# microsoft/NOTSOFAR1-Challenge

Measured on AMD Instinct MI355X. Metric: CSS real-time-factor (sep. audio sec/wall sec) on 7-ch 16 kHz, higher is better.
Workload: dtype f32 (float32 operands on v_mfma_f32_32x32x2_f32 in every Linear layer, attention product and transform: the reference's own operand precision; MVDR covariance / solve f64)

## Files before the change

include/css_mi355.h:

```cpp
#ifndef CSS_MI355_H
#define CSS_MI355_H

#include <stddef.h>
#include <stdint.h>

#ifdef __cplusplus
extern "C" {
#endif
#if defined(__GNUC__) || defined(__clang__)
#pragma GCC visibility push(default)
#endif

typedef struct css_ctx* css_handle_t;

typedef enum css_status {
    CSS_OK = 0,
    CSS_ERR_INVALID_ARG = -1,
    CSS_ERR_HIP = -2,
    CSS_ERR_ZERO_WEIGHT = -3,
    CSS_ERR_MASK_FLOOR = -4,
    CSS_ERR_SHAPE = -5,
    CSS_ERR_STATE = -6,
    CSS_ERR_NO_DEVICE = -7,
    CSS_ERR_WEIGHT_WINDOW = -8,
// ... 79 lines not shown
    CSS_BUF_ACT_FINAL = 11,
    CSS_BUF_Y = 12,
    CSS_BUF_WAV = 13,
    CSS_BUF_HIDDEN = 14,
    CSS_BUF_WTA_OVERRIDE = 15,
    CSS_BUF_LEVEL = 16
} css_buffer;

const char* css_version(void);
const char* css_last_error(css_handle_t h);
int css_device_count(void);

int64_t css_blob_num_floats(const CssModelDesc* desc);

int css_create(const CssModelDesc* desc, const float* blob_host, int64_t blob_floats, int device,
               void* stream, int32_t max_batch_segments, css_handle_t* out);
int css_destroy(css_handle_t h);
int css_get_stream(css_handle_t h, void** stream_out);
int css_set_lanes(css_handle_t h, int lanes);
int css_get_lanes(css_handle_t h);
enum css_tuning {
    CSS_TUNE_TAIL_PIECES = 0,
    CSS_TUNE_OUT_MAPPED = 1,
    CSS_TUNE_TAIL_PER_UNIT = 2,
    CSS_TUNE_MVDR_ON_LANES = 3,
    CSS_TUNE_PIPELINE_DEVICE = 4,
    CSS_TUNE_GROUP_LANES = 5,
    CSS_TUNE_GROUP_TRANSFORM_ON_MAIN = 6,
    CSS_TUNE_GROUP_MVDR_ON_LANES = 7,
    CSS_TUNE_GROUP_OUT_DMA = 8,
    CSS_TUNE_F32_GEMM = 9,
    CSS_TUNE_SPLIT_BATCH_ROWS = 10,
    CSS_TUNE_F32_LANE_ROWS = 11,
    CSS_TUNE_COUNT = 12
};
int css_set_tuning(css_handle_t h, int which, int value);
int css_host_alloc(size_t bytes, void** out);
int css_host_free(void* p);

int css_plan(const CssModelDesc* desc, const CssRunCfg* cfg, int64_t n_samples, CssPlan* out);
int css_pit_scan(const double* costs, int64_t n_boundaries, int32_t num_spks, int32_t* perms);

typedef struct CssCfgSeconds {
    double segment_size_sec;
    double hop_size_sec;
    double seg_weight_m0_sec;
    double seg_weight_m1_sec;
    double activity_dilation_sec;
    double activity_erosion_sec;
    double activity_th;
    double mask_floor_db;
    int32_t mc_mvdr, stitching_loss , stitching_input , normalize_segment_power;
} CssCfgSeconds;
int css_make_run_cfg(const CssModelDesc* desc, const CssCfgSeconds* cfg, int32_t fs, CssRunCfg* out, float* windows, int64_t cap);

int css_run(css_handle_t h, const float* pcm_host, int64_t n_samples, int32_t n_ch, const CssRunCfg* cfg,
            float* wav_host, int64_t wav_capacity_per_stream);
int css_run_enqueue(css_handle_t h, const float* pcm_host, int64_t n_samples, int32_t n_ch, const CssRunCfg* cfg,
                    float* wav_host, int64_t cap);
int css_set_queue_group(css_handle_t h, int max_sessions);
int css_wait(css_handle_t h);
int css_wait_sessions(css_handle_t h, int64_t n);
int css_run_device(css_handle_t h, const float* pcm_dev, int64_t n_samples, int32_t n_ch, const CssRunCfg* cfg,
                   float* wav_dev, int64_t wav_capacity_per_stream);
int css_run_pcm16(css_handle_t h, const int16_t* const* planes_host, int64_t n_samples, int32_t n_ch, const CssRunCfg* cfg,
                  int16_t* wav_pcm16_host, int64_t wav_capacity_per_stream, float* peaks_host);
int css_run_enqueue_pcm16(css_handle_t h, const int16_t* const* planes_host, int64_t n_samples, int32_t n_ch, const CssRunCfg* cfg,
// ... 129 lines not shown
```

notsofar1-challenge_amd/_lib.py:

```python
from __future__ import annotations

import ctypes as C
import os
from typing import Optional

import numpy as np

_HERE = os.path.dirname(os.path.abspath(__file__))
LIB_PATH = os.environ.get("CSS_MI355_LIBRARY") or os.path.join(_HERE, "libcss_mi355.so")


class CssLibraryError(RuntimeError):
    pass


class CssError(RuntimeError):
    def __init__(self, code: int, text: str):
        super().__init__(f"css_mi355 error {code}: {text}")
        self.code = code
        self.text = text


CSS_OK, CSS_ERR_INVALID_ARG, CSS_ERR_HIP, CSS_ERR_ZERO_WEIGHT, CSS_ERR_MASK_FLOOR = 0, -1, -2, -3, -4
CSS_ERR_SHAPE, CSS_ERR_STATE, CSS_ERR_NO_DEVICE, CSS_ERR_WEIGHT_WINDOW, CSS_ERR_RANGE = -5, -6, -7, -8, -9
# ... 359 lines not shown
        blob = np.ascontiguousarray(blob, dtype=np.float32)
        need = lib.css_blob_num_floats(C.byref(self._cdesc))
        if need != blob.size:
            raise CssError(CSS_ERR_INVALID_ARG, f"weight blob has {blob.size} floats, library expects {need}")
        h = C.c_void_p()
        rc = lib.css_create(C.byref(self._cdesc), _np_ptr(blob), blob.size, int(device),
                            C.c_void_p(stream) if stream else None, int(max_batch_segments), C.byref(h))
        if rc != CSS_OK:
            raise CssError(rc, lib.css_last_error(None).decode("utf-8", "replace"))
        self.h = h
        self.device = device

    def close(self):
        if getattr(self, "h", None):
            self.lib.css_destroy(self.h)
            self.h = None

    def __del__(self):
        try:
            self.close()
        except Exception:
            pass

    def stream_ptr(self) -> int:
        p = C.c_void_p()
        check(self.h, self.lib.css_get_stream(self.h, C.byref(p)))
        return int(p.value or 0)

    def set_lanes(self, lanes: int):
        check(self.h, self.lib.css_set_lanes(self.h, int(lanes)))

    def set_tuning(self, which, value: int):
        idx = {"tail_pieces": 0, "out_mapped": 1, "tail_per_unit": 2, "mvdr_on_lanes": 3, "pipeline_device": 4,
               "group_lanes": 5, "group_transform_on_main": 6, "group_mvdr_on_lanes": 7, "group_out_dma": 8, "f32_gemm": 9, "split_batch_rows": 10, "f32_lane_rows": 11}[which] if isinstance(which, str) else int(which)
        check(self.h, self.lib.css_set_tuning(self.h, idx, int(value)))

    def set_queue_group(self, max_sessions: int):
        check(self.h, self.lib.css_set_queue_group(self.h, int(max_sessions)))

    def lanes(self) -> int:
        return int(self.lib.css_get_lanes(self.h))

    def run(self, pcm: np.ndarray, cfg: RunCfg, out: Optional[np.ndarray] = None) -> np.ndarray:
        pcm = np.ascontiguousarray(pcm, dtype=np.float32)
        n, c = pcm.shape
        p = plan(self.desc, cfg, n)
        if out is None:
            out = np.empty((self.desc.num_spks, p.n_out), dtype=np.float32)
        assert out.dtype == np.float32 and out.ndim == 2 and out.shape[0] == self.desc.num_spks and out.shape[1] >= p.n_out \
            and out.strides[1] == 4
        check(self.h, self.lib.css_run(self.h, _np_ptr(pcm), n, c, C.byref(cfg.c), _np_ptr(out), out.strides[0] // 4))
        return out[:, :p.n_out]

    def run_enqueue(self, pcm: np.ndarray, cfg: RunCfg, out: np.ndarray) -> np.ndarray:
        assert pcm.dtype == np.float32 and pcm.flags.c_contiguous and pcm.ndim == 2
        n, c = pcm.shape
        p = plan(self.desc, cfg, n)
        assert out.dtype == np.float32 and out.ndim == 2 and out.shape[0] == self.desc.num_spks and out.shape[1] >= p.n_out \
            and out.strides[1] == 4
        self._queued_keep = getattr(self, "_queued_keep", []) + [(pcm, out, cfg)]
        check(self.h, self.lib.css_run_enqueue(self.h, _np_ptr(pcm), n, c, C.byref(cfg.c), _np_ptr(out), out.strides[0] // 4))
        return out[:, :p.n_out]

    def wait(self):
        try:
            check(self.h, self.lib.css_wait(self.h))
        finally:
# ... 293 lines not shown
```

notsofar1-challenge_amd/csrc/api_ctx.hpp:

```cpp
#pragma once
#include "../../include/css_mi355.h"

#include <algorithm>
#include <cmath>
#include <cstdlib>
#include <cstdio>
#include <cstring>
#include <chrono>
#include <functional>
#include <string>
#include <vector>

#include <dlfcn.h>
#include <mutex>

#include "kernels.hpp"
#include "lsap.hpp"

using namespace css;

enum ProfCat : int {
    CSS_PROF_DEINTERLEAVE = 0, CSS_PROF_STFT, CSS_PROF_FEATURES, CSS_PROF_LINEAR, CSS_PROF_LAYERNORM, CSS_PROF_ATTENTION,
    CSS_PROF_CONV, CSS_PROF_SCM, CSS_PROF_MVDR_SOLVE, CSS_PROF_BEAMFORM, CSS_PROF_PIT, CSS_PROF_OLA_MASKS, CSS_PROF_GATE,
    CSS_PROF_OLA_STFT, CSS_PROF_ISTFT_GEMM, CSS_PROF_WAVE_OLA, CSS_PROF_ENCODE, CSS_PROF_COUNT
// ... 85 lines not shown
    bool split_ok = true;
    float* wsplit = nullptr;
    float* dft_split = nullptr;
    float* wfrag = nullptr;
    float* dft_tiled = nullptr;
    float* head_tiled = nullptr;
    DevBuf pe_frag[2];
    int pe_frag_T[2] = {0, 0};
    float* stft_tab = nullptr;
    bool fft512 = true;
    float* dft_fwd = nullptr;
    int Lp = 0, ovl = 2;
    float* dft_inv_t = nullptr;

    std::vector<float> w_on_device;
    DevBuf pcm_in, feat, hx, hu, ht, qkv, qkf, ctxb, masks, segw, stage, in16, pcm_f, enc, level, mel_tab, mel_work;
    static constexpr int MAX_GROUP = 8;
    std::vector<SessState> slots;
    int group_limit = MAX_GROUP;
    static constexpr int MAX_LANES = 4;
    int lanes = 3;
    hipStream_t lane_stream[MAX_LANES] = {};
    hipEvent_t ev_fork = nullptr, ev_join[MAX_LANES] = {};
    DevBuf lfeat[MAX_LANES], lhx[MAX_LANES], lhu[MAX_LANES], lht[MAX_LANES], lqkv[MAX_LANES], lqkf[MAX_LANES], lctx[MAX_LANES];
    int64_t last_batch_tokens = 0;
    int mel_bands = 0;
    unsigned int* range_flag_dev = nullptr;
    unsigned int* range_flag_host = nullptr;
    bool range_fallback = true;
    int64_t range_fallbacks = 0;
    int range_last = 0;
    hipStream_t copy_stream = nullptr;
    hipStream_t tail_stream = nullptr;
    int tune[CSS_TUNE_COUNT] = {1, 0, 0, 1, 0, 2, 1, 0, 1, 0, 24576, 14000};
    const void* mapped_key = nullptr;
    void* mapped_val = nullptr;
    int queued = 0;
    int64_t pass_no = 0;
    hipEvent_t pcm_free[2] = {nullptr, nullptr};
    hipEvent_t pass_end[4] = {nullptr, nullptr, nullptr, nullptr};
    hipEvent_t level_free[2] = {nullptr, nullptr};
    hipEvent_t tail_end = nullptr;
    bool tail_pending = false;
    bool piped_now = false;
    int last_piped = -1;
    struct QueuedSession {
        const float* pcm; int64_t n; int32_t n_ch; CssRunCfg cfg; float* wav; int64_t cap;
        std::vector<const int16_t*> planes; int16_t* wav16; float* peaks;
        float* wav_mapped;
        std::vector<float> w;
        QueuedSession(const float* pcm_, const int16_t* const* planes_, int64_t n_, int32_t n_ch_, const CssRunCfg& c, float* wav_,
                      int16_t* wav16_, float* peaks_, int64_t cap_, float* mapped_)
            : pcm(pcm_), n(n_), n_ch(n_ch_), cfg(c), wav(wav_), cap(cap_), wav16(wav16_), peaks(peaks_), wav_mapped(mapped_) {
            if (planes_) planes.assign(planes_, planes_ + n_ch_);
            const size_t T = (size_t)std::max(c.segment_frames, 0);
            w.resize(3 * T);
            if (T && c.w_first && c.w_mid && c.w_last) {
                std::memcpy(w.data(), c.w_first, T * sizeof(float));
                std::memcpy(w.data() + T, c.w_mid, T * sizeof(float));
                std::memcpy(w.data() + 2 * T, c.w_last, T * sizeof(float));
            }
        }
        bool pcm16() const { return !planes.empty(); }
        CssRunCfg own_cfg() const {
            CssRunCfg c = cfg;
            const size_t T = w.size() / 3;
            c.w_first = w.data(); c.w_mid = w.data() + T; c.w_last = w.data() + 2 * T;
// ... 153 lines not shown
```

notsofar1-challenge_amd/csrc/api_stages.hip:

```cpp
#include "api_ctx.hpp"

int check_run_args(css_handle_t h, int64_t n_samples, int32_t n_ch, const CssRunCfg* cfg, CssPlan* plan_out) {
    if (!h || !cfg) return fail(h, CSS_ERR_INVALID_ARG, "null argument");
    if (n_ch != h->d.num_mics)
        return fail(h, CSS_ERR_SHAPE, "input has " + std::to_string(n_ch) + " channels, the model expects " + std::to_string(h->d.num_mics));
    if (!cfg->w_first || !cfg->w_mid || !cfg->w_last) return fail(h, CSS_ERR_INVALID_ARG, "segment weights missing");
    if (cfg->mask_floor > 1.0f || cfg->mask_floor < 0.f) return fail(h, CSS_ERR_MASK_FLOOR, "mask_floor_db must be <= 0");
    const int T = cfg->segment_frames, hop = cfg->hop_frames;
    if (T < 2 || T > CSS_MAX_SEGMENT_FRAMES)
        return fail(h, CSS_ERR_INVALID_ARG, "segment_frames must be in [2, " + std::to_string(CSS_MAX_SEGMENT_FRAMES) + "]");
    if (cfg->stitching_loss < 0 || cfg->stitching_loss > 1 || cfg->stitching_input < 0 || cfg->stitching_input > 1)
        return fail(h, CSS_ERR_INVALID_ARG, "unexpected stitching_loss / stitching_input");
    if (hop <= 0 || hop >= T) return fail(h, CSS_ERR_INVALID_ARG, "hop_frames must satisfy 1 <= hop < T (at least one frame of overlap for the stitching cost, css.py:276)");
    CssPlan p{};
    if (plan_impl(h->d, *cfg, n_samples, &p) != CSS_OK) return fail(h, CSS_ERR_INVALID_ARG, "bad segment configuration");
    if (p.zero_weight) return fail(h, CSS_ERR_ZERO_WEIGHT, "zero weights found. check hop_size, segment_size or m0, m1");
    *plan_out = p;
    return CSS_OK;
}

int begin_impl(css_handle_t h, int64_t n_samples, int32_t n_ch, const CssRunCfg* cfg) {
    CssPlan p{};
    int rc0 = check_run_args(h, n_samples, n_ch, cfg, &p);
    if (rc0 != CSS_OK) return rc0;
// ... 229 lines not shown
                       const float* w2, const float* b2) {
            if (with_ln) { CSS_PROF(CSS_PROF_LAYERNORM, st); launch_layernorm(xin, sp ? nullptr : u, sp ? u : nullptr, lnw, lnb, M, D, 0, st); }
            gemm(h, lin(u, D, w1, b1, t1, FF, FF, D, ACT_RELU, FF), st);
            GemmArgs g = lin(t1, FF, w2, b2, x, D, D, FF, ACT_NONE, 0);
            g.residual = xin; g.ldr = D; g.alpha = 0.5f;
            gemm(h, g, st);
        };
        ffn(l == 0, x, b.ffi_ln_w, b.ffi_ln_b, b.ffi_w1, b.ffi_b1, b.ffi_w2, b.ffi_b2);
        { CSS_PROF(CSS_PROF_LAYERNORM, st); launch_layernorm(x, sp ? nullptr : u, sp ? u : nullptr, b.att_ln_w, b.att_ln_b, M, D, 0, st); }
        const bool long_seg = T > 512 || css_force_long_path();
        {
            GemmArgs g = lin(u, D, b.wqkv, b.bqkv, qkv, 3 * D, 3 * D, D, ACT_NONE, long_seg ? 0 : 3 * D);
            if (sp && !long_seg) { g.frag_out = qkf; g.frag_D = D; g.frag_T = T; g.frag_heads = d.attention_heads; g.frag_invT = 1.0f / T; }
            gemm(h, g, st);
        }
        {
            CSS_PROF(CSS_PROF_ATTENTION, st);
            if (long_seg) {
                if (!launch_relpos_attention_long(qkv, W.pe_k, cb, nb, T, D, d.attention_heads, d.maxlen, sp, st)) return CSS_ERR_INVALID_ARG;
            } else {
                launch_relpos_attention(qkv, sp ? qkf : nullptr, (const float*)h->pe_frag[sp].p, cb, nb, T, D, d.attention_heads, d.maxlen, sp, sp, st);
            }
        }
        {
            GemmArgs g = lin(cb, D, b.wo, b.bo, x, D, D, D, ACT_NONE, 0);
            g.residual = x; g.ldr = D; g.alpha = 1.f;
            gemm(h, g, st);
        }
        const float* xc = cb;
        bool ffo_ln = false;
        {
        CSS_PROF(CSS_PROF_CONV, st);
        if (!launch_conv_module(x, cb, b.conv_ln_w, b.conv_ln_b, b.pw, b.dw_wt, b.dw_b, b.bn_alpha, b.bn_beta, b.ffo_ln_w,
                                b.ffo_ln_b, sp ? nullptr : u, sp ? u : nullptr, nb, T, D, d.kernel_size, st)) {
            launch_ln_glu(x, u, b.conv_ln_w, b.conv_ln_b, b.pw, M, D, st);
            launch_dwconv(u, x, b.dw_wt, b.dw_b, b.bn_alpha, b.bn_beta, b.pw, nb, T, D, d.kernel_size, st);
            xc = x;
            ffo_ln = true;
        }
        }
        ffn(ffo_ln, xc, b.ffo_ln_w, b.ffo_ln_b, b.ffo_w1, b.ffo_b1, b.ffo_w2, b.ffo_b2);
        if (!last) {
            const BlockWeights& nb_ = W.blocks[l + 1];
            { CSS_PROF(CSS_PROF_LAYERNORM, st); launch_layernorm2(x, x, b.fin_ln_w, b.fin_ln_b, sp ? nullptr : u, sp ? u : nullptr, nb_.ffi_ln_w, nb_.ffi_ln_b, M, D, st); }
        } else {
            { CSS_PROF(CSS_PROF_LAYERNORM, st); launch_layernorm(x, x, sp ? u : nullptr, b.fin_ln_w, b.fin_ln_b, M, D, 0, st); }
        }
    }
    if (ph_hi <= d.num_blocks) return CSS_OK;
    GemmArgs g{};
    const int nout = F * (d.num_spks + d.num_nois);
    if (sp) {
        g.A = u; g.lda = D; g.strideA = 0;
        g.B = h->head_tiled; g.ldb = D; g.strideB = 0; g.b_tiled = 1;
        g.C = io.masks + s0 * T; g.ldc = io.mask_ld; g.strideC = 0; g.c_transposed = 1;
        g.M = M; g.N = nout; g.K = D; g.batch = 1;
        g.bias = W.head_b; g.bias_along_m = 0; g.act = ACT_SIGMOID; g.residual = nullptr; g.alpha = 1.f;
        g.split_in = 1; g.concurrent = concurrent ? 1 : 0;
        g.range_flag = h->range_flag_dev;
    } else {
        g.A = WS(W.head_w); g.lda = D; g.strideA = 0;
        g.B = sp ? u : x; g.ldb = D; g.strideB = 0;
        g.C = io.masks + s0 * T; g.ldc = io.mask_ld; g.strideC = 0;
        g.M = nout; g.N = M; g.K = D; g.batch = 1;
        g.bias = W.head_b; g.bias_along_m = 1; g.act = ACT_SIGMOID; g.residual = nullptr; g.alpha = 1.f;
        g.split_in = sp;
        g.range_flag = sp ? h->range_flag_dev : nullptr;
// ... 573 lines not shown
```

notsofar1-challenge_amd/csrc/encoder.hip:

```cpp
#include "kernels.hpp"
#include "split_f16.hpp"

namespace css {

typedef float f32x16 __attribute__((ext_vector_type(16)));
typedef _Float16 f16x8 __attribute__((ext_vector_type(8)));

template <int CTRL>
__device__ __forceinline__ float dpp_addf(float v) {
    return v + __int_as_float(__builtin_amdgcn_update_dpp(0, __float_as_int(v), CTRL, 0xf, 0xf, false));
}
__device__ __forceinline__ float wave_sum(float v) {
    v = dpp_addf<0xB1>(v);
    v = dpp_addf<0x4E>(v);
    v = dpp_addf<0x141>(v);
    v = dpp_addf<0x140>(v);
    const float r0 = __int_as_float(__builtin_amdgcn_readlane(__float_as_int(v), 0));
    const float r1 = __int_as_float(__builtin_amdgcn_readlane(__float_as_int(v), 16));
    const float r2 = __int_as_float(__builtin_amdgcn_readlane(__float_as_int(v), 32));
    const float r3 = __int_as_float(__builtin_amdgcn_readlane(__float_as_int(v), 48));
    return (r0 + r1) + (r2 + r3);
}

#ifndef CSS_LN_ROWS
// ... 144 lines not shown
#pragma clang loop unroll(full)
    for (int p = 0; p < RUN + TAPS - 1; ++p) {
        const int t = t0 + p - PAD;
        const float v = (t >= 0 && t < T) ? zs[(int64_t)t * D] : 0.f;
#pragma clang loop unroll(full)
        for (int j = (p - (TAPS - 1) > 0 ? p - (TAPS - 1) : 0); j <= (p < RUN - 1 ? p : RUN - 1); ++j)
            acc[j] = fmaf(wk[p - j], v, acc[j]);
    }
    const float bb = dwb[ch], al = alpha[ch], be = beta[ch], w2 = pw[4], c2 = pw[5];
    float* hs = h + (int64_t)seg * T * D + ch;
#pragma unroll
    for (int j = 0; j < RUN; ++j) {
        const int t = t0 + j;
        if (t < T) {
            const float y = fmaxf((acc[j] + bb) * al + be, 0.f);
            hs[(int64_t)t * D] += w2 * y + c2;
        }
    }
}

void launch_dwconv(const float* z, float* h, const float* dw_wt, const float* dw_b, const float* bn_alpha,
                   const float* bn_beta, const float* pw, int nseg, int T, int D, int taps, hipStream_t s) {
    constexpr int RUN = 31;
    const int runs = (T + RUN - 1) / RUN;
    const dim3 grid((D + 255) / 256, nseg * runs), block(256);
    if (taps == 33)
        hipLaunchKernelGGL((dwconv_kernel<33, RUN>), grid, block, 0, s, z, h, dw_wt, dw_b, bn_alpha, bn_beta, pw, T, D, runs);
    else if (taps == 31)
        hipLaunchKernelGGL((dwconv_kernel<31, RUN>), grid, block, 0, s, z, h, dw_wt, dw_b, bn_alpha, bn_beta, pw, T, D, runs);
    else if (taps == 17)
        hipLaunchKernelGGL((dwconv_kernel<17, RUN>), grid, block, 0, s, z, h, dw_wt, dw_b, bn_alpha, bn_beta, pw, T, D, runs);
}

template <int NV, int TAPS, int RUN, int HV>
__global__ __launch_bounds__(256 * NV * HV) void conv_module_kernel(const float* __restrict__ x_in, float* __restrict__ x_out,
                                                              const float* __restrict__ lnw, const float* __restrict__ lnb,
                                                              const float* __restrict__ pw, const float* __restrict__ wt,
                                                              const float* __restrict__ dwb, const float* __restrict__ alpha,
                                                              const float* __restrict__ beta,
                                                              const float* __restrict__ ln2w, const float* __restrict__ ln2b,
                                                              float* __restrict__ z, float* __restrict__ zs, int T, int runs_per_seg) {
    constexpr int D = 256 * NV, PAD = (TAPS - 1) / 2, ROWS = RUN + TAPS - 1, NW = 4 * NV * HV, JH = (RUN + HV - 1) / HV;
    extern __shared__ __attribute__((aligned(16))) float tile[];
    const int item = css_xcd_item((int)blockIdx.x, (int)gridDim.x);
    const int seg = item / runs_per_seg, run = item % runs_per_seg;
    const int t0 = run * RUN;
    const int wave = threadIdx.x >> 6, lane = threadIdx.x & 63;
    const float p0 = pw[0], p1 = pw[1], p2 = pw[2], p3 = pw[3];
    const int ch = threadIdx.x % D, j0 = (threadIdx.x / D) * JH;
    float wk[TAPS];
#pragma clang loop unroll(full)
    for (int k = 0; k < TAPS; ++k) wk[k] = wt[k * D + ch];
    const float bb = dwb[ch], al = alpha[ch], be_ = beta[ch], w2 = pw[4], c2 = pw[5];
    const float* xs = x_in + (int64_t)seg * T * D + ch;
    float xres[JH];
#pragma clang loop unroll(full)
    for (int j = 0; j < JH; ++j) xres[j] = xs[(int64_t)min(t0 + j0 + j, T - 1) * D];
    constexpr int RPW = (ROWS + NW - 1) / NW;
    float4 v[RPW][NV];
#pragma unroll
    for (int i = 0; i < RPW; ++i) {
        const int p = wave + i * NW, t = t0 + p - PAD;
        const bool ok = p < ROWS && t >= 0 && t < T;
        const float4* xr = reinterpret_cast<const float4*>(x_in + ((int64_t)seg * T + (ok ? t : 0)) * D);
#pragma unroll
        for (int j = 0; j < NV; ++j) v[i][j] = ok ? xr[lane + 64 * j] : make_float4(0.f, 0.f, 0.f, 0.f);
    }
#pragma unroll
    for (int i = 0; i < RPW; ++i) {
        const int p = wave + i * NW, t = t0 + p - PAD;
        if (p >= ROWS) break;
        float4* dst = reinterpret_cast<float4*>(tile + p * D);
        if (t < 0 || t >= T) {
#pragma unroll
            for (int j = 0; j < NV; ++j) dst[lane + 64 * j] = make_float4(0.f, 0.f, 0.f, 0.f);
            continue;
        }
        float s = 0.f;
#pragma unroll
        for (int j = 0; j < NV; ++j) s += (v[i][j].x + v[i][j].y) + (v[i][j].z + v[i][j].w);
        const float mean = wave_sum(s) * (1.0f / D);
        float q = 0.f;
#pragma unroll
        for (int j = 0; j < NV; ++j) {
            v[i][j].x -= mean; v[i][j].y -= mean; v[i][j].z -= mean; v[i][j].w -= mean;
            q += (v[i][j].x * v[i][j].x + v[i][j].y * v[i][j].y) + (v[i][j].z * v[i][j].z + v[i][j].w * v[i][j].w);
        }
        const float rstd = 1.0f / sqrtf(wave_sum(q) * (1.0f / D) + 1e-5f);
#pragma unroll
        for (int j = 0; j < NV; ++j) {
            const float4 g = reinterpret_cast<const float4*>(lnw)[lane + 64 * j];
            const float4 be = reinterpret_cast<const float4*>(lnb)[lane + 64 * j];
            float o[4] = {v[i][j].x * rstd * g.x + be.x, v[i][j].y * rstd * g.y + be.y, v[i][j].z * rstd * g.z + be.z,
                          v[i][j].w * rstd * g.w + be.w};
#pragma unroll
            for (int e = 0; e < 4; ++e) {
                const float z = p2 * o[e] + p3;
                o[e] = (p0 * o[e] + p1) * __builtin_amdgcn_rcpf(1.0f + __builtin_amdgcn_exp2f(z * -1.44269504088896341f));
            }
            dst[lane + 64 * j] = make_float4(o[0], o[1], o[2], o[3]);
        }
    }
    __syncthreads();
    float acc[JH];
#pragma clang loop unroll(full)
    for (int j = 0; j < JH; ++j) acc[j] = 0.f;
#pragma clang loop unroll(full)
    for (int pp = 0; pp < JH + TAPS - 1; ++pp) {
        const float zv = tile[min(j0 + pp, ROWS - 1) * D + ch];
#pragma clang loop unroll(full)
        for (int j = (pp - (TAPS - 1) > 0 ? pp - (TAPS - 1) : 0); j <= (pp < JH - 1 ? pp : JH - 1); ++j)
            acc[j] = fmaf(wk[pp - j], zv, acc[j]);
    }
    __syncthreads();
#pragma unroll
    for (int j = 0; j < JH; ++j) {
        const float y = fmaxf((acc[j] + bb) * al + be_, 0.f);
        if (j0 + j < RUN) tile[(j0 + j) * D + ch] = xres[j] + (w2 * y + c2);
    }
    __syncthreads();
    for (int j = wave; j < RUN && t0 + j < T; j += NW) {
        const int64_t row = (int64_t)seg * T + t0 + j;
        float4 r[NV];
        float s = 0.f;
#pragma unroll
        for (int i = 0; i < NV; ++i) {
            r[i] = reinterpret_cast<const float4*>(tile + j * D)[lane + 64 * i];
            reinterpret_cast<float4*>(x_out + row * D)[lane + 64 * i] = r[i];
            s += (r[i].x + r[i].y) + (r[i].z + r[i].w);
        }
        if (!z && !zs) continue;
        const float mean = wave_sum(s) * (1.0f / D);
        float q = 0.f;
#pragma unroll
        for (int i = 0; i < NV; ++i) {
            r[i].x -= mean; r[i].y -= mean; r[i].z -= mean; r[i].w -= mean;
            q += (r[i].x * r[i].x + r[i].y * r[i].y) + (r[i].z * r[i].z + r[i].w * r[i].w);
        }
        const float rstd = 1.0f / sqrtf(wave_sum(q) * (1.0f / D) + 1e-5f);
#pragma unroll
        for (int i = 0; i < NV; ++i) {
            const float4 g = reinterpret_cast<const float4*>(ln2w)[lane + 64 * i];
            const float4 be = reinterpret_cast<const float4*>(ln2b)[lane + 64 * i];
            const float4 o = make_float4(r[i].x * rstd * g.x + be.x, r[i].y * rstd * g.y + be.y, r[i].z * rstd * g.z + be.z,
                                         r[i].w * rstd * g.w + be.w);
            if (z) reinterpret_cast<float4*>(z + row * D)[lane + 64 * i] = o;
            if (zs) split_store4(reinterpret_cast<_Float16*>(zs + row * D), 4 * (lane + 64 * i), o.x, o.y, o.z, o.w);
        }
    }
}

bool launch_conv_module(const float* x_in, float* x_out, const float* ln_w, const float* ln_b, const float* pw,
                        const float* dw_wt, const float* dw_b, const float* bn_alpha, const float* bn_beta,
                        const float* ln2_w, const float* ln2_b, float* z, float* z_split, int nseg, int T,
                        int D, int taps, hipStream_t s) {
#ifndef CSS_CONV_RUN
#define CSS_CONV_RUN 31
#endif
    constexpr int RUN = CSS_CONV_RUN;
    if (taps != 33 || (D != 256 && D != 512)) return false;
    const int runs = (T + RUN - 1) / RUN;
    const size_t lds = (size_t)(RUN + 32) * D * sizeof(float);
    const void* fn = D == 512 ? reinterpret_cast<const void*>(&conv_module_kernel<2, 33, RUN, 2>)
                              : reinterpret_cast<const void*>(&conv_module_kernel<1, 33, RUN, 2>);
    if (hipFuncSetAttribute(fn, hipFuncAttributeMaxDynamicSharedMemorySize, 160 * 1024) != hipSuccess) {
        (void)hipGetLastError();
        return false;
    }
    if (D == 512)
        hipLaunchKernelGGL((conv_module_kernel<2, 33, RUN, 2>), dim3(nseg * runs), dim3(1024), lds, s, x_in, x_out, ln_w, ln_b, pw, dw_wt,
                           dw_b, bn_alpha, bn_beta, ln2_w, ln2_b, z, z_split, T, runs);
    else
        hipLaunchKernelGGL((conv_module_kernel<1, 33, RUN, 2>), dim3(nseg * runs), dim3(512), lds, s, x_in, x_out, ln_w, ln_b, pw, dw_wt,
                           dw_b, bn_alpha, bn_beta, ln2_w, ln2_b, z, z_split, T, runs);
    return true;
}

template <int NJT, bool QKS, bool FRAG, int W>
__global__ __launch_bounds__(64 * W, (NJT <= 7 ? 2 : 1)) void relpos_attn_kernel(const float* __restrict__ qkv, const float* __restrict__ qkf,
                                                         const float* __restrict__ pe,
                                                         float* __restrict__ ctx, int T, int D, int maxlen,
                                                         int split_out, int heads, int n_items) {
    constexpr int DK = 64;
    constexpr int LDR = 98;
    const int wv = W > 1 ? __builtin_amdgcn_readfirstlane((int)(threadIdx.x >> 6)) : 0;
    __shared__ __attribute__((aligned(16))) float lds_all[W][32 * LDR];
    float (&lds)[32 * LDR] = lds_all[wv];
    const int item = css_xcd_item((int)blockIdx.x, (int)gridDim.x) * W + wv;
    if (item >= n_items) return;
    const int qt = item % NJT, head = (item / NJT) % heads, seg = item / (NJT * heads);
    const int lane = threadIdx.x & 63, c = lane & 31, h = lane >> 5;
    const int ld = 3 * D;
    const float* qb = qkv + (int64_t)seg * T * ld + head * DK;
    const float* kb = qb + D;
    const float* vb = qb + 2 * D;
    const int i0 = qt * 32;
    const int iq = min(i0 + c, T - 1);

    float4 q[8];
#define CSS_ATT_LOAD8(dst, rowptr)                                                                      \
    _Pragma("unroll") for (int ch = 0; ch < 8; ++ch)                                                    \
        dst[ch] = *reinterpret_cast<const float4*>((rowptr) + (QKS ? ((ch >> 2) * 32 + ((ch >> 1) & 1) * 8 + (ch & 1) * 16) : 8 * ch) + 4 * h);
    const float4* qkt = reinterpret_cast<const float4*>(qkf) +
                        ((int64_t)(seg * heads + head) * NJT) * (2 * 8 * 64) + lane;
    if constexpr (FRAG) {
#pragma unroll
        for (int ch = 0; ch < 8; ++ch) q[ch] = qkt[(qt * 2 + 0) * 512 + ch * 64];
// ... 430 lines not shown
```

notsofar1-challenge_amd/csrc/kernels.hpp:

```cpp
#pragma once
#include <hip/hip_runtime.h>
#include <stdint.h>

namespace css {

enum GemmAct : int { ACT_NONE = 0, ACT_RELU = 1, ACT_SIGMOID = 2 };

struct GemmArgs {
    const float* A; int64_t lda; int64_t strideA;
    const float* B; int64_t ldb; int64_t strideB;
    float* C; int64_t ldc; int64_t strideC;
    int M, N, K, batch;
    const float* bias;
    int bias_along_m;
    int act;
    const float* residual;
    int64_t ldr;
    float alpha;
    int split_in;
    int split_out;
    int b_tiled;
    int b_frag32;
    const float* B_rows;
    int concurrent;
    int nt_store;
    float* frag_out;
    int frag_D, frag_T, frag_heads;
    float frag_invT;
    int tile_rows;
    int narrow_epilogue;
    unsigned int* range_flag;
    int layout;
    int m_fastest;
    int c_transposed;
};
void launch_gemm(const GemmArgs& g, hipStream_t s);
bool launch_gemm_f32(const GemmArgs& g, hipStream_t s, int forced_tm);
void launch_f32_fragments(const float* src, int64_t ld_src, float* dst, int N, int K, hipStream_t s);
void launch_gemm_split(const GemmArgs& g, hipStream_t s);
void launch_gemm_split_wd(const GemmArgs& g, hipStream_t s);
void launch_split_convert_tiled(const float* src, int64_t ld_src, float* dst, int N, int K, hipStream_t s);
void launch_split_convert(const float* src, int64_t ld_src, float* dst, int64_t rows, int K, int Kp, hipStream_t s);

void launch_layernorm(const float* x, float* y, float* y_split, const float* w, const float* b, int rows, int D,
                      int relu, hipStream_t s);
void launch_layernorm2(const float* x, float* y, const float* w1, const float* b1, float* z, float* z_split,
                       const float* w2, const float* b2, int rows, int D, hipStream_t s);
void launch_ln_glu(const float* x, float* z, const float* w, const float* b, const float* pw, int rows, int D,
                   hipStream_t s);
void launch_dwconv(const float* z, float* h, const float* dw_wt, const float* dw_b, const float* bn_alpha,
                   const float* bn_beta, const float* pw, int nseg, int T, int D, int taps, hipStream_t s);
bool launch_conv_module(const float* x_in, float* x_out, const float* ln_w, const float* ln_b, const float* pw,
                        const float* dw_wt, const float* dw_b, const float* bn_alpha, const float* bn_beta,
                        const float* ln2_w, const float* ln2_b, float* z, float* z_split, int nseg, int T,
                        int D, int taps, hipStream_t s);
inline int pe_fragment_tiles(int T) { return 2 * ((T + 31) / 32); }
void launch_pe_fragments(const float* pe, float* frag, int T, int maxlen, int split, hipStream_t s);
inline int64_t qk_fragment_floats(int64_t nseg, int T, int H) { return nseg * H * ((T + 31) / 32) * 2 * 8 * 64 * 4; }
void launch_relpos_attention(const float* qkv, const float* qk_frag, const float* pe_frag, float* ctx, int nseg, int T, int D,
                             int H, int maxlen, int qk_split, int split_out, hipStream_t s);
bool launch_relpos_attention_long(const float* qkv, const float* pe, float* ctx, int nseg, int T, int D, int H, int maxlen,
                                  int split_out, hipStream_t s);

size_t stft_table_floats();
void stft_build_tables(float* host, int window = 0);
bool launch_stft_fft(const float* x, int64_t x_stride, int C, int64_t t_lo, int64_t t_hi, const float* tables, float* out,
                     int64_t row_ld, hipStream_t s, float* phase = nullptr);

__device__ __forceinline__ int css_xcd_item(int L, int n) {
    const int q = n >> 3, rem = n & 7, xcd = L & 7;
    return xcd * q + (xcd < rem ? xcd : rem) + (L >> 3);
}

#define CSS_PHASE_NEG_REAL (-3.14159250259399414f)
__device__ __forceinline__ float css_phase_of(float re, float im) {
    return (im == 0.f && re < 0.f) ? CSS_PHASE_NEG_REAL : atan2f(im, re);
}

void launch_deinterleave(const float* pcm, float* pcm_cm, int64_t n, int C, int64_t n_pad, int64_t i_lo, int64_t i_hi,
                         int split_out, hipStream_t s);
void launch_pcm_peak_f32(const float* x, int64_t count, unsigned int* peak, hipStream_t s);
void launch_pcm_peak_i16(const int16_t* x, int64_t count, unsigned int* peak, hipStream_t s);
void launch_pcm16_to_float(const int16_t* planes, float* pcm, int64_t n, int C, hipStream_t s);
void launch_pcm16_to_channel_major(const int16_t* planes, float* pcm_cm, int64_t n, int C, int64_t n_pad, int64_t i_lo,
                                   int64_t i_hi, hipStream_t s);
void launch_encode_pcm16(const float* wav, int S, int64_t n, unsigned int* peak_bits, int16_t* out, int64_t out_ld,
                         hipStream_t s);
bool css_force_long_path();
// ... 122 lines not shown
```

Before: 7295.

## Stream multiple conv runs per block with ring-buffered GLU rows and prefetch

The fused conformer conv-module kernel now lets each block process a span of consecutive runs of a segment. The block keeps GLU-activated rows in a ring buffer in LDS, so the 32-row halo shared by adjacent runs is not recomputed (LayerNorm+GLU) or reloaded. Input rows for the next run are prefetched into registers while the current run is convolved and written out. Span is picked automatically so the grid keeps at least ~240 blocks; the trade-off is fewer blocks and serialised runs within a block, plus extra register pressure from the prefetch buffers.

```diff
diff --git a/include/css_mi355.h b/include/css_mi355.h
--- a/include/css_mi355.h
+++ b/include/css_mi355.h
@@ -135,7 +135,8 @@
     CSS_TUNE_F32_GEMM = 9,
     CSS_TUNE_SPLIT_BATCH_ROWS = 10,
     CSS_TUNE_F32_LANE_ROWS = 11,
-    CSS_TUNE_COUNT = 12
+    CSS_TUNE_CONV_SPAN = 12,
+    CSS_TUNE_COUNT = 13
 };
 int css_set_tuning(css_handle_t h, int which, int value);
 int css_host_alloc(size_t bytes, void** out);
diff --git a/notsofar1-challenge_amd/_lib.py b/notsofar1-challenge_amd/_lib.py
--- a/notsofar1-challenge_amd/_lib.py
+++ b/notsofar1-challenge_amd/_lib.py
@@ -415,7 +415,7 @@
 
     def set_tuning(self, which, value: int):
         idx = {"tail_pieces": 0, "out_mapped": 1, "tail_per_unit": 2, "mvdr_on_lanes": 3, "pipeline_device": 4,
-               "group_lanes": 5, "group_transform_on_main": 6, "group_mvdr_on_lanes": 7, "group_out_dma": 8, "f32_gemm": 9, "split_batch_rows": 10, "f32_lane_rows": 11}[which] if isinstance(which, str) else int(which)
+               "group_lanes": 5, "group_transform_on_main": 6, "group_mvdr_on_lanes": 7, "group_out_dma": 8, "f32_gemm": 9, "split_batch_rows": 10, "f32_lane_rows": 11, "conv_span": 12}[which] if isinstance(which, str) else int(which)
         check(self.h, self.lib.css_set_tuning(self.h, idx, int(value)))
 
     def set_queue_group(self, max_sessions: int):
diff --git a/notsofar1-challenge_amd/csrc/api_ctx.hpp b/notsofar1-challenge_amd/csrc/api_ctx.hpp
--- a/notsofar1-challenge_amd/csrc/api_ctx.hpp
+++ b/notsofar1-challenge_amd/csrc/api_ctx.hpp
@@ -141,7 +141,7 @@
     int range_last = 0;
     hipStream_t copy_stream = nullptr;
     hipStream_t tail_stream = nullptr;
-    int tune[CSS_TUNE_COUNT] = {1, 0, 0, 1, 0, 2, 1, 0, 1, 0, 24576, 14000};
+    int tune[CSS_TUNE_COUNT] = {1, 0, 0, 1, 0, 2, 1, 0, 1, 0, 24576, 14000, 0};
     const void* mapped_key = nullptr;
     void* mapped_val = nullptr;
     int queued = 0;
diff --git a/notsofar1-challenge_amd/csrc/api_stages.hip b/notsofar1-challenge_amd/csrc/api_stages.hip
--- a/notsofar1-challenge_amd/csrc/api_stages.hip
+++ b/notsofar1-challenge_amd/csrc/api_stages.hip
@@ -285,7 +285,7 @@
         {
         CSS_PROF(CSS_PROF_CONV, st);
         if (!launch_conv_module(x, cb, b.conv_ln_w, b.conv_ln_b, b.pw, b.dw_wt, b.dw_b, b.bn_alpha, b.bn_beta, b.ffo_ln_w,
-                                b.ffo_ln_b, sp ? nullptr : u, sp ? u : nullptr, nb, T, D, d.kernel_size, st)) {
+                                b.ffo_ln_b, sp ? nullptr : u, sp ? u : nullptr, nb, T, D, d.kernel_size, h->tune[CSS_TUNE_CONV_SPAN], st)) {
             launch_ln_glu(x, u, b.conv_ln_w, b.conv_ln_b, b.pw, M, D, st);
             launch_dwconv(u, x, b.dw_wt, b.dw_b, b.bn_alpha, b.bn_beta, b.pw, nb, T, D, d.kernel_size, st);
             xc = x;
diff --git a/notsofar1-challenge_amd/csrc/encoder.hip b/notsofar1-challenge_amd/csrc/encoder.hip
--- a/notsofar1-challenge_amd/csrc/encoder.hip
+++ b/notsofar1-challenge_amd/csrc/encoder.hip
@@ -200,6 +200,37 @@
         hipLaunchKernelGGL((dwconv_kernel<17, RUN>), grid, block, 0, s, z, h, dw_wt, dw_b, bn_alpha, bn_beta, pw, T, D, runs);
 }
 
+template <int NV>
+__device__ __forceinline__ void conv_glu_row(float4 (&v)[NV], float4* __restrict__ dst, unsigned lane, const float* __restrict__ lnw,
+                                             const float* __restrict__ lnb, float p0, float p1, float p2, float p3) {
+    constexpr int D = 256 * NV;
+    asm volatile("" : "+v"(lane));
+    float s = 0.f;
+#pragma unroll
+    for (int j = 0; j < NV; ++j) s += (v[j].x + v[j].y) + (v[j].z + v[j].w);
+    const float mean = wave_sum(s) * (1.0f / D);
+    float q = 0.f;
+#pragma unroll
+    for (int j = 0; j < NV; ++j) {
+        v[j].x -= mean; v[j].y -= mean; v[j].z -= mean; v[j].w -= mean;
+        q += (v[j].x * v[j].x + v[j].y * v[j].y) + (v[j].z * v[j].z + v[j].w * v[j].w);
+    }
+    const float rstd = 1.0f / sqrtf(wave_sum(q) * (1.0f / D) + 1e-5f);
+#pragma unroll
+    for (int j = 0; j < NV; ++j) {
+        const float4 g = reinterpret_cast<const float4*>(lnw)[lane + 64u * j];
+        const float4 be = reinterpret_cast<const float4*>(lnb)[lane + 64u * j];
+        float o[4] = {v[j].x * rstd * g.x + be.x, v[j].y * rstd * g.y + be.y, v[j].z * rstd * g.z + be.z,
+                      v[j].w * rstd * g.w + be.w};
+#pragma unroll
+        for (int e = 0; e < 4; ++e) {
+            const float z = p2 * o[e] + p3;
+            o[e] = (p0 * o[e] + p1) * __builtin_amdgcn_rcpf(1.0f + __builtin_amdgcn_exp2f(z * -1.44269504088896341f));
+        }
+        dst[lane + 64u * j] = make_float4(o[0], o[1], o[2], o[3]);
+    }
+}
+
 template <int NV, int TAPS, int RUN, int HV>
 __global__ __launch_bounds__(256 * NV * HV) void conv_module_kernel(const float* __restrict__ x_in, float* __restrict__ x_out,
                                                               const float* __restrict__ lnw, const float* __restrict__ lnb,
@@ -207,140 +238,189 @@
                                                               const float* __restrict__ dwb, const float* __restrict__ alpha,
                                                               const float* __restrict__ beta,
                                                               const float* __restrict__ ln2w, const float* __restrict__ ln2b,
-                                                              float* __restrict__ z, float* __restrict__ zs, int T, int runs_per_seg) {
+                                                              float* __restrict__ z, float* __restrict__ zs, int T, int runs_per_seg,
+                                                              int span) {
     constexpr int D = 256 * NV, PAD = (TAPS - 1) / 2, ROWS = RUN + TAPS - 1, NW = 4 * NV * HV, JH = (RUN + HV - 1) / HV;
+    constexpr int RPW = (ROWS + NW - 1) / NW;
+    constexpr int NPW = (RUN + NW - 1) / NW;
     extern __shared__ __attribute__((aligned(16))) float tile[];
     const int item = css_xcd_item((int)blockIdx.x, (int)gridDim.x);
-    const int seg = item / runs_per_seg, run = item % runs_per_seg;
-    const int t0 = run * RUN;
-    const int wave = threadIdx.x >> 6, lane = threadIdx.x & 63;
+    const int spans_per_seg = (runs_per_seg + span - 1) / span;
+    const int seg = item / spans_per_seg, run0 = (item % spans_per_seg) * span;
+    const int nrun = min(span, runs_per_seg - run0);
+    const int wave = __builtin_amdgcn_readfirstlane(threadIdx.x >> 6);
+    const unsigned lane_ = threadIdx.x & 63, lane = lane_;
     const float p0 = pw[0], p1 = pw[1], p2 = pw[2], p3 = pw[3];
-    const int ch = threadIdx.x % D, j0 = (threadIdx.x / D) * JH;
+    const unsigned ch = threadIdx.x % D;
+    const int j0 = __builtin_amdgcn_readfirstlane((threadIdx.x / D) * JH);
     float wk[TAPS];
 #pragma clang loop unroll(full)
-    for (int k = 0; k < TAPS; ++k) wk[k] = wt[k * D + ch];
+    for (int k = 0; k < TAPS; ++k) wk[k] = (wt + k * D)[ch];
     const float bb = dwb[ch], al = alpha[ch], be_ = beta[ch], w2 = pw[4], c2 = pw[5];
-    const float* xs = x_in + (int64_t)seg * T * D + ch;
+    const float* xs = x_in + (int64_t)seg * T * D;
     float xres[JH];
-#pragma clang loop unroll(full)
-    for (int j = 0; j < JH; ++j) xres[j] = xs[(int64_t)min(t0 + j0 + j, T - 1) * D];
-    constexpr int RPW = (ROWS + NW - 1) / NW;
-    float4 v[RPW][NV];
-#pragma unroll
-    for (int i = 0; i < RPW; ++i) {
-        const int p = wave + i * NW, t = t0 + p - PAD;
-        const bool ok = p < ROWS && t >= 0 && t < T;
-        const float4* xr = reinterpret_cast<const float4*>(x_in + ((int64_t)seg * T + (ok ? t : 0)) * D);
-#pragma unroll
-        for (int j = 0; j < NV; ++j) v[i][j] = ok ? xr[lane + 64 * j] : make_float4(0.f, 0.f, 0.f, 0.f);
-    }
-#pragma unroll
-    for (int i = 0; i < RPW; ++i) {
-        const int p = wave + i * NW, t = t0 + p - PAD;
-        if (p >= ROWS) break;
-        float4* dst = reinterpret_cast<float4*>(tile + p * D);
-        if (t < 0 || t >= T) {
-#pragma unroll
-            for (int j = 0; j < NV; ++j) dst[lane + 64 * j] = make_float4(0.f, 0.f, 0.f, 0.f);
-            continue;
-        }
-        float s = 0.f;
-#pragma unroll
-        for (int j = 0; j < NV; ++j) s += (v[i][j].x + v[i][j].y) + (v[i][j].z + v[i][j].w);
-        const float mean = wave_sum(s) * (1.0f / D);
-        float q = 0.f;
-#pragma unroll
-        for (int j = 0; j < NV; ++j) {
-            v[i][j].x -= mean; v[i][j].y -= mean; v[i][j].z -= mean; v[i][j].w -= mean;
-            q += (v[i][j].x * v[i][j].x + v[i][j].y * v[i][j].y) + (v[i][j].z * v[i][j].z + v[i][j].w * v[i][j].w);
-        }
-        const float rstd = 1.0f / sqrtf(wave_sum(q) * (1.0f / D) + 1e-5f);
-#pragma unroll
-        for (int j = 0; j < NV; ++j) {
-            const float4 g = reinterpret_cast<const float4*>(lnw)[lane + 64 * j];
-            const float4 be = reinterpret_cast<const float4*>(lnb)[lane + 64 * j];
-            float o[4] = {v[i][j].x * rstd * g.x + be.x, v[i][j].y * rstd * g.y + be.y, v[i][j].z * rstd * g.z + be.z,
-                          v[i][j].w * rstd * g.w + be.w};
-#pragma unroll
-            for (int e = 0; e < 4; ++e) {
-                const float z = p2 * o[e] + p3;
-                o[e] = (p0 * o[e] + p1) * __builtin_amdgcn_rcpf(1.0f + __builtin_amdgcn_exp2f(z * -1.44269504088896341f));
+    {
+        const int t0 = run0 * RUN;
+#pragma clang loop unroll(full)
+        for (int j = 0; j < JH; ++j) xres[j] = (xs + (int64_t)min(t0 + j0 + j, T - 1) * D)[ch];
+        float4 v[RPW][NV];
+#pragma unroll
+        for (int i = 0; i < RPW; ++i) {
+            const int p = wave + i * NW, t = t0 + p - PAD;
+            const bool ok = p < ROWS && t >= 0 && t < T;
+            const float4* xr = reinterpret_cast<const float4*>(x_in + ((int64_t)seg * T + (ok ? t : 0)) * D);
+#pragma unroll
+            for (int j = 0; j < NV; ++j) v[i][j] = ok ? xr[lane + 64u * j] : make_float4(0.f, 0.f, 0.f, 0.f);
+        }
+#pragma unroll
+        for (int i = 0; i < RPW; ++i) {
+            const int p = wave + i * NW, t = t0 + p - PAD;
+            if (p >= ROWS) break;
+            float4* dst = reinterpret_cast<float4*>(tile + p * D);
+            if (t < 0 || t >= T) {
+#pragma unroll
+                for (int j = 0; j < NV; ++j) dst[lane + 64u * j] = make_float4(0.f, 0.f, 0.f, 0.f);
+                continue;
             }
-            dst[lane + 64 * j] = make_float4(o[0], o[1], o[2], o[3]);
-        }
-    }
-    __syncthreads();
-    float acc[JH];
-#pragma clang loop unroll(full)
-    for (int j = 0; j < JH; ++j) acc[j] = 0.f;
-#pragma clang loop unroll(full)
-    for (int pp = 0; pp < JH + TAPS - 1; ++pp) {
-        const float zv = tile[min(j0 + pp, ROWS - 1) * D + ch];
-#pragma clang loop unroll(full)
-        for (int j = (pp - (TAPS - 1) > 0 ? pp - (TAPS - 1) : 0); j <= (pp < JH - 1 ? pp : JH - 1); ++j)
-            acc[j] = fmaf(wk[pp - j], zv, acc[j]);
-    }
-    __syncthreads();
-#pragma unroll
-    for (int j = 0; j < JH; ++j) {
-        const float y = fmaxf((acc[j] + bb) * al + be_, 0.f);
-        if (j0 + j < RUN) tile[(j0 + j) * D + ch] = xres[j] + (w2 * y + c2);
-    }
-    __syncthreads();
-    for (int j = wave; j < RUN && t0 + j < T; j += NW) {
-        const int64_t row = (int64_t)seg * T + t0 + j;
-        float4 r[NV];
-        float s = 0.f;
-#pragma unroll
-        for (int i = 0; i < NV; ++i) {
-            r[i] = reinterpret_cast<const float4*>(tile + j * D)[lane + 64 * i];
-            reinterpret_cast<float4*>(x_out + row * D)[lane + 64 * i] = r[i];
-            s += (r[i].x + r[i].y) + (r[i].z + r[i].w);
-        }
-        if (!z && !zs) continue;
-        const float mean = wave_sum(s) * (1.0f / D);
-        float q = 0.f;
-#pragma unroll
-        for (int i = 0; i < NV; ++i) {
-            r[i].x -= mean; r[i].y -= mean; r[i].z -= mean; r[i].w -= mean;
-            q += (r[i].x * r[i].x + r[i].y * r[i].y) + (r[i].z * r[i].z + r[i].w * r[i].w);
-        }
-        const float rstd = 1.0f / sqrtf(wave_sum(q) * (1.0f / D) + 1e-5f);
-#pragma unroll
-        for (int i = 0; i < NV; ++i) {
-            const float4 g = reinterpret_cast<const float4*>(ln2w)[lane + 64 * i];
-            const float4 be = reinterpret_cast<const float4*>(ln2b)[lane + 64 * i];
-            const float4 o = make_float4(r[i].x * rstd * g.x + be.x, r[i].y * rstd * g.y + be.y, r[i].z * rstd * g.z + be.z,
-                                         r[i].w * rstd * g.w + be.w);
-            if (z) reinterpret_cast<float4*>(z + row * D)[lane + 64 * i] = o;
-            if (zs) split_store4(reinterpret_cast<_Float16*>(zs + row * D), 4 * (lane + 64 * i), o.x, o.y, o.z, o.w);
-        }
-    }
+            conv_glu_row<NV>(v[i], dst, lane, lnw, lnb, p0, p1, p2, p3);
+        }
+    }
+    float4 nv[NPW][NV];
+    const auto request_rows = [&](int t_first, bool any) {
+#pragma unroll
+        for (int i = 0; i < NPW; ++i) {
+            const int j = wave + i * NW, t = t_first + j;
+            const bool ok = any && j < RUN && t < T;
+            const float4* xr = reinterpret_cast<const float4*>(x_in + ((int64_t)seg * T + (ok ? t : 0)) * D);
+#pragma unroll
+            for (int k = 0; k < NV; ++k) nv[i][k] = ok ? xr[lane + 64u * k] : make_float4(0.f, 0.f, 0.f, 0.f);
+        }
+    };
+    request_rows(run0 * RUN + RUN + PAD, nrun > 1);
+    int base = 0;
+    for (int ri = 0;; ++ri) {
+        const int t0 = (run0 + ri) * RUN;
+        const bool more = ri + 1 < nrun;
+        __syncthreads();
+        static_assert(HV <= 2, "base + j0 must stay below 2 * ROWS");
+        const int start = base + j0 >= ROWS ? base + j0 - ROWS : base + j0;
+        float acc[JH];
+#pragma clang loop unroll(full)
+        for (int j = 0; j < JH; ++j) acc[j] = 0.f;
+        int rt = start;
+#pragma clang loop unroll(full)
+        for (int pp = 0; pp < JH + TAPS - 1; ++pp) {
+            const float zv = tile[rt * D + ch];
+            rt = rt + 1 == ROWS ? 0 : rt + 1;
+#pragma clang loop unroll(full)
+            for (int j = (pp - (TAPS - 1) > 0 ? pp - (TAPS - 1) : 0); j <= (pp < JH - 1 ? pp : JH - 1); ++j)
+                acc[j] = fmaf(wk[pp - j], zv, acc[j]);
+        }
+        __syncthreads();
+        int ro = start;
+        asm volatile("" : "+s"(ro));
+#pragma unroll
+        for (int j = 0; j < JH; ++j) {
+            const float y = fmaxf((acc[j] + bb) * al + be_, 0.f);
+            if (j0 + j < RUN) tile[ro * D + ch] = xres[j] + (w2 * y + c2);
+            ro = ro + 1 == ROWS ? 0 : ro + 1;
+        }
+        if (more) {
+            unsigned chn = ch;
+            asm volatile("" : "+v"(chn));
+#pragma clang loop unroll(full)
+            for (int j = 0; j < JH; ++j) xres[j] = (xs + (int64_t)min(t0 + RUN + j0 + j, T - 1) * D)[chn];
+        }
+        __syncthreads();
+#pragma unroll
+        for (int i = 0; i < NPW; ++i) {
+            const int j = wave + i * NW;
+            if (j >= RUN) break;
+            int r = base + j;
+            r = r >= ROWS ? r - ROWS : r;
+            float4* slot = reinterpret_cast<float4*>(tile + r * D);
+            unsigned lane = lane_;
+            asm volatile("" : "+v"(lane));
+            if (t0 + j < T) {
+                const int64_t row = (int64_t)seg * T + t0 + j;
+                float4 o4[NV];
+                float s = 0.f;
+#pragma unroll
+                for (int k = 0; k < NV; ++k) {
+                    o4[k] = slot[lane + 64u * k];
+                    reinterpret_cast<float4*>(x_out + row * D)[lane + 64u * k] = o4[k];
+                    s += (o4[k].x + o4[k].y) + (o4[k].z + o4[k].w);
+                }
+                if (z || zs) {
+                    const float mean = wave_sum(s) * (1.0f / D);
+                    float q = 0.f;
+#pragma unroll
+                    for (int k = 0; k < NV; ++k) {
+                        o4[k].x -= mean; o4[k].y -= mean; o4[k].z -= mean; o4[k].w -= mean;
+                        q += (o4[k].x * o4[k].x + o4[k].y * o4[k].y) + (o4[k].z * o4[k].z + o4[k].w * o4[k].w);
+                    }
+                    const float rstd = 1.0f / sqrtf(wave_sum(q) * (1.0f / D) + 1e-5f);
+#pragma unroll
+                    for (int k = 0; k < NV; ++k) {
+                        const float4 g = reinterpret_cast<const float4*>(ln2w)[lane + 64u * k];
+                        const float4 be = reinterpret_cast<const float4*>(ln2b)[lane + 64u * k];
+                        const float4 o = make_float4(o4[k].x * rstd * g.x + be.x, o4[k].y * rstd * g.y + be.y,
+                                                     o4[k].z * rstd * g.z + be.z, o4[k].w * rstd * g.w + be.w);
+                        if (z) reinterpret_cast<float4*>(z + row * D)[lane + 64u * k] = o;
+                        if (zs) split_store4(reinterpret_cast<_Float16*>(zs + row * D), 4 * (int)(lane + 64u * k), o.x, o.y, o.z, o.w);
+                    }
+                }
+            }
+            if (more) {
+                if (t0 + RUN + PAD + j < T) {
+                    conv_glu_row<NV>(nv[i], slot, lane, lnw, lnb, p0, p1, p2, p3);
+                } else {
+#pragma unroll
+                    for (int k = 0; k < NV; ++k) slot[lane + 64u * k] = make_float4(0.f, 0.f, 0.f, 0.f);
+                }
+            }
+        }
+        if (!more) break;
+        request_rows(t0 + 2 * RUN + PAD, ri + 2 < nrun);
+        base = base + RUN >= ROWS ? base + RUN - ROWS : base + RUN;
+    }
+}
+
+static int conv_auto_span(int nseg, int runs) {
+    constexpr int FILL = 240;
+    int span = 1;
+    for (int s = 2; s <= runs; ++s)
+        if (nseg * ((runs + s - 1) / s) >= FILL) span = s;
+    return span;
 }
 
 bool launch_conv_module(const float* x_in, float* x_out, const float* ln_w, const float* ln_b, const float* pw,
                         const float* dw_wt, const float* dw_b, const float* bn_alpha, const float* bn_beta,
                         const float* ln2_w, const float* ln2_b, float* z, float* z_split, int nseg, int T,
-                        int D, int taps, hipStream_t s) {
+                        int D, int taps, int span, hipStream_t s) {
 #ifndef CSS_CONV_RUN
 #define CSS_CONV_RUN 31
 #endif
     constexpr int RUN = CSS_CONV_RUN;
+    constexpr size_t LDS_CAP = 160 * 1024;
+    static_assert((size_t)(RUN + 32) * 512 * sizeof(float) <= LDS_CAP, "the ring of GLU rows must fit the CU's LDS");
     if (taps != 33 || (D != 256 && D != 512)) return false;
     const int runs = (T + RUN - 1) / RUN;
+    span = span <= 0 ? conv_auto_span(nseg, runs) : std::min(span, runs);
+    const int blocks = nseg * ((runs + span - 1) / span);
     const size_t lds = (size_t)(RUN + 32) * D * sizeof(float);
     const void* fn = D == 512 ? reinterpret_cast<const void*>(&conv_module_kernel<2, 33, RUN, 2>)
                               : reinterpret_cast<const void*>(&conv_module_kernel<1, 33, RUN, 2>);
-    if (hipFuncSetAttribute(fn, hipFuncAttributeMaxDynamicSharedMemorySize, 160 * 1024) != hipSuccess) {
+    if (hipFuncSetAttribute(fn, hipFuncAttributeMaxDynamicSharedMemorySize, (int)LDS_CAP) != hipSuccess) {
         (void)hipGetLastError();
         return false;
     }
     if (D == 512)
-        hipLaunchKernelGGL((conv_module_kernel<2, 33, RUN, 2>), dim3(nseg * runs), dim3(1024), lds, s, x_in, x_out, ln_w, ln_b, pw, dw_wt,
-                           dw_b, bn_alpha, bn_beta, ln2_w, ln2_b, z, z_split, T, runs);
+        hipLaunchKernelGGL((conv_module_kernel<2, 33, RUN, 2>), dim3(blocks), dim3(1024), lds, s, x_in, x_out, ln_w, ln_b, pw, dw_wt,
+                           dw_b, bn_alpha, bn_beta, ln2_w, ln2_b, z, z_split, T, runs, span);
     else
-        hipLaunchKernelGGL((conv_module_kernel<1, 33, RUN, 2>), dim3(nseg * runs), dim3(512), lds, s, x_in, x_out, ln_w, ln_b, pw, dw_wt,
-                           dw_b, bn_alpha, bn_beta, ln2_w, ln2_b, z, z_split, T, runs);
+        hipLaunchKernelGGL((conv_module_kernel<1, 33, RUN, 2>), dim3(blocks), dim3(512), lds, s, x_in, x_out, ln_w, ln_b, pw, dw_wt,
+                           dw_b, bn_alpha, bn_beta, ln2_w, ln2_b, z, z_split, T, runs, span);
     return true;
 }
 
diff --git a/notsofar1-challenge_amd/csrc/kernels.hpp b/notsofar1-challenge_amd/csrc/kernels.hpp
--- a/notsofar1-challenge_amd/csrc/kernels.hpp
+++ b/notsofar1-challenge_amd/csrc/kernels.hpp
@@ -53,7 +53,7 @@
 bool launch_conv_module(const float* x_in, float* x_out, const float* ln_w, const float* ln_b, const float* pw,
                         const float* dw_wt, const float* dw_b, const float* bn_alpha, const float* bn_beta,
                         const float* ln2_w, const float* ln2_b, float* z, float* z_split, int nseg, int T,
-                        int D, int taps, hipStream_t s);
+                        int D, int taps, int span, hipStream_t s);
 inline int pe_fragment_tiles(int T) { return 2 * ((T + 31) / 32); }
 void launch_pe_fragments(const float* pe, float* frag, int T, int maxlen, int split, hipStream_t s);
 inline int64_t qk_fragment_floats(int64_t nseg, int T, int H) { return nseg * H * ((T + 31) / 32) * 2 * 8 * 64 * 4; }
```

Measured after the change: 7231. Within noise of the previous version (-0.9%).
